# tzjtatata/Myriad

Measured on AMD Instinct MI355X. Metric: images/sec fine-tune step (Vicuna-7B + LoRA-style adapters, 224px), higher is better.
Workload: dtype bf16

## Files before the change

include/myriad_hip.h:

```cpp
#ifndef MYRIAD_HIP_H
#define MYRIAD_HIP_H
#include <stdint.h>

#ifdef __cplusplus
extern "C" {
#endif

typedef struct ihipStream_t* mh_stream_t;

#define MH_OK 0
#define MH_ERR_ARG (-1)
#define MH_ERR_LAUNCH (-2)
#define MH_ERR_UNSUPPORTED (-3)

#define MH_GEMM_OUT_F32 1
#define MH_GEMM_GELU 2
#define MH_GEMM_REGSTAGE 4

int mh_gemm_bf16_nt(const void* A, int lda, const void* B, int ldb, void* C, int ldc, int M, int N, int K,
                    const float* bias, const float* residual, int ldr, int flags, float alpha, mh_stream_t s);

int mh_gemm_plan(int M, int N, int K, int flags, int* kernel, int* splits);

int mh_prof_start(int capacity, mh_stream_t s);
double mh_prof_overhead_ms(void);
int mh_prof_stop(int* meta, float* ms, int cap, mh_stream_t s);

int mh_gemm_residual_rmsnorm(const void* A, int lda, const void* B, int ldb, float* H, int ldh, const float* residual,
                             int ldr, const float* norm_w, float eps, void* Y, long ldy, int M, int N, int K,
                             mh_stream_t s);

int mh_gemm_residual_layernorm(const void* A, int lda, const void* B, int ldb, float* H, int ldh, const float* bias,
                               const float* residual, int ldr, const float* norm_w, const float* norm_b, float eps, void* Y,
                               int M, int N, int K, mh_stream_t s);
int mh_gemm_rmsnorm_bwd(const void* A, int lda, const void* B, int ldb, float* dy_buf, const float* x, const float* w,
                        const float* dres, float* dx, void* dx_bf16, int M, int N, int K, float eps, mh_stream_t s);
int mh_gemm_layernorm_bwd(const void* A, int lda, const void* B, int ldb, float* dy_buf, const float* x, const float* w,
                          const float* dres, float* dx, void* dx_bf16, float* dgamma, float* dbeta, int accumulate, float* ws,
                          long ws_floats, int M, int N, int K, float eps, mh_stream_t s);

int mh_set_workspace(void* ptr, long bytes);
int mh_set_stream_workspace(mh_stream_t stream, void* ptr, long bytes);
long mh_gemm_splitk_ws_floats(int M, int N, int splits);
int mh_gemm_bf16_nt_splitk(const void* A, int lda, const void* B, int ldb, float* C, int ldc, int M, int N, int K,
                           int splits, float* ws, mh_stream_t s);

int mh_attn_fwd(const void* q, const void* k, const void* v, void* o, float* lse, const float* bias,
                const int* kv_len, int B, int H, int Sq, int Sk, int D, long q_bs, int ldq, long k_bs, int ldk,
                long v_bs, int ldv, long o_bs, int ldo, float scale, int causal, mh_stream_t s);
int mh_attn_fwd_dropout(const void* q, const void* k, const void* v, void* o, float* lse, int B, int H, int Sq, int Sk, int D,
                        long q_bs, int ldq, long k_bs, int ldk, long v_bs, int ldv, long o_bs, int ldo, float scale,
                        float drop_p, unsigned long long seed, mh_stream_t s);
int mh_attn_bwd_dropout(const void* q, const void* k, const void* v, const void* o, const void* dout, const float* lse,
                        float* delta_ws, void* dq, void* dk, void* dv, int B, int H, int Sq, int Sk, int D, long q_bs, int ldq,
                        long k_bs, int ldk, long v_bs, int ldv, long o_bs, int ldo, long do_bs, int lddo, long dq_bs,
                        int lddq, long dk_bs, int lddk, long dv_bs, int lddv, float scale, float drop_p,
                        unsigned long long seed, mh_stream_t s);
int mh_attn_bwd(const void* q, const void* k, const void* v, const void* o, const void* dout, const float* lse,
                float* delta_ws , void* dq, void* dk, void* dv, const float* bias,
                const int* kv_len, int B, int H, int Sq, int Sk, int D, long q_bs, int ldq, long k_bs, int ldk,
                long v_bs, int ldv, long o_bs, int ldo, long do_bs, int lddo, long dq_bs, int lddq, long dk_bs,
                int lddk, long dv_bs, int lddv, float scale, int causal, mh_stream_t s);

int mh_attn_rope_supported(int S, int D);
int mh_attn_rope_fwd(const void* qkv, int ld, void* o, int ldo, float* lse, const int* pos, const float* cos_tab,
                     const float* sin_tab, const int* kv_len, int B, int H, int S, int D, float scale, mh_stream_t s);
int mh_attn_rope_bwd(const void* qkv, int ld, const void* o, int ldo, const void* dout, int ldd, const float* lse,
                     void* dqkv, const int* pos, const float* cos_tab, const float* sin_tab, const int* kv_len,
                     int B, int H, int S, int D, float scale, mh_stream_t s);
int mh_gemm_attn_rope_bwd(const void* A, int lda, const void* Bw, int ldb, void* do_buf, int K, const void* qkv,
                          int ld, const void* o, int ldo, const float* lse, void* dqkv, const int* pos,
                          const float* cos_tab, const float* sin_tab, const int* kv_len, int B, int H, int S,
                          int D, float scale, mh_stream_t s);

int mh_rmsnorm_fwd(const float* x, const float* w, void* y_bf16, long ldy, int M, int D, float eps, mh_stream_t s);
int mh_rmsnorm_bwd(const float* dy, const float* x, const float* w, const float* dres, float* dx, void* dx_bf16,
                   int M, int D, float eps, mh_stream_t s);
int mh_layernorm_fwd(const float* x, const float* w, const float* b, void* y_bf16, float* y_f32, int M, int D,
                     float eps, mh_stream_t s);
int mh_layernorm_bwd(const float* dy, const float* x, const float* w, const float* dres, float* dx, void* dx_bf16,
                     int M, int D, float eps, mh_stream_t s);
long mh_layernorm_param_grads_ws_floats(int M, int D);
int mh_layernorm_param_grads(const float* dy, const float* x, float* dgamma, float* dbeta, int M, int D, float eps,
                             int accumulate, float p_out, unsigned long long seed_out, float* ws, long ws_floats,
                             mh_stream_t s);
int mh_layernorm_fwd_dropout(const float* z, const float* res, const float* w, const float* b, float* x_out, void* y_bf16,
                             float* y_f32, int M, int D, float eps, float p_in, unsigned long long seed_in, float p_out,
                             unsigned long long seed_out, mh_stream_t s);
int mh_layernorm_bwd_dropout(const float* dy, const float* x, const float* w, float* dx, void* dz_bf16, int M, int D,
                             float eps, float p_in, unsigned long long seed_in, float p_out, unsigned long long seed_out,
                             mh_stream_t s);
int mh_dropout_keep_mask(float* out, long n, float p, unsigned long long seed, mh_stream_t s);
int mh_drop_path_residual_layernorm(const float* h, const float* y, const int* slot_in, int K_in, float scale, const float* w,
                                    const float* b, const int* slot_out, int K_out, float* h_out, void* xn_bf16, int B, int N,
                                    int D, float eps, mh_stream_t s);
int mh_drop_path_layernorm_bwd(const float* dy, const float* x, const float* w, const float* dres, const int* slot_in, int K_in,
                               const int* slot_out, int K_out, float out_scale, float* dx, void* dx_bf16, int B, int N, int D,
                               float eps, mh_stream_t s);
int mh_drop_path_gather_scale(const float* src, const int* slot_out, int K_out, float scale, void* dst_bf16, int B, int N, int D,
                              mh_stream_t s);
long mh_drop_path_param_grads_ws_floats(int K, int N, int D);
int mh_drop_path_layernorm_param_grads(const float* dy, const float* x, const int* slot_in, int K_in, float* dgamma, float* dbeta,
                                       int B, int N, int D, float eps, int accumulate, float* ws, long ws_floats, mh_stream_t s);
long mh_gemm_tn_wgrad_ws_floats(int M, int N, int K, int splits);
int mh_gemm_tn_wgrad_auto_splits(int M, int N, int K);
int mh_gemm_tn_wgrad(const void* dy, long lddy, const void* x, long ldx, float* out, long ldo, float* bias, int M, int N, int K,
                     int accumulate, int splits, float* ws, long ws_floats, mh_stream_t s);

int mh_rope_inplace(void* x, int ld, int col0, int n_tok, int n_heads, int head_dim, const int* pos,
                    const float* cos_tab, const float* sin_tab, float sign, mh_stream_t s);
int mh_silu_mul_fwd(const void* gu, void* h, int M, int I, mh_stream_t s);
int mh_silu_mul_bwd(const void* dh, const void* gu, void* dgu, int M, int I, mh_stream_t s);
int mh_silu_mul_fwd_blk(const void* gu, void* h, int M, int I, int blk, mh_stream_t s);
int mh_silu_mul_bwd_blk(const void* dh, const void* gu, void* dgu, int M, int I, int blk, mh_stream_t s);
int mh_gemm_swiglu_fwd(const void* X, int ldx, const void* Wgu, int ldw, void* gu, int ldgu, void* act, int ldact, int M,
                       int I, int K, mh_stream_t s);
int mh_gemm_swiglu_bwd(const void* dH, int lddh, const void* WdT, int ldw, const void* gu, int ldgu, void* dgu, int lddgu,
                       void* dact_buf, int M, int I, int K, mh_stream_t s);
int mh_gelu_fwd(const void* x, void* y, long n, mh_stream_t s);
int mh_gelu_bwd(const void* dy, const void* x, void* dx, long n, mh_stream_t s);
int mh_gemm_gelu_fwd(const void* X, int ldx, const void* W, int ldw, const float* bias, void* pre, int ldpre, void* act, int ldact,
                     int M, int N, int K, mh_stream_t s);
int mh_gemm_gelu_bwd(const void* dY, int lddy, const void* WT, int ldw, const void* pre, int ldpre, void* dpre, int lddpre,
                     void* dact_buf, int M, int N, int K, mh_stream_t s);

int mh_dropout_bf16(const void* x, long ldx, void* y, long ldy, long rows, int cols, float p, unsigned long long seed,
                    mh_stream_t s);
int mh_dropout_add_f32(const float* dy, long lddy, float* acc, long ldacc, long rows, int cols, float p,
                       unsigned long long seed, mh_stream_t s);

int mh_lora_down(const void* x, long ldx, const float* A, void* border, long ldo, int M, int D, int R2, float s, float p,
                 unsigned long long seed, mh_stream_t st);
int mh_lora_dx(const float* dx_ext, long ld, const float* A, float* out, int M, int D, int R2, float s, float p,
               unsigned long long seed, mh_stream_t st);
int mh_rmsnorm_lora_down(const float* h, long ldh, const float* norm_w, float eps, const float* A, void* x_ext, long ldx, int M,
                         int D, int R2, float s, mh_stream_t st);
int mh_gemm_lora_dx(const void* A, int lda, const void* Bw, int ldb, float* dx_ext_buf, const float* loraA, float* dxn,
                    float* border_out, int M, int D, int K, int R2, float s, float p, unsigned long long seed, mh_stream_t stream);
int mh_gemm_lora_rmsnorm_bwd(const void* A, int lda, const void* Bw, int ldb, float* dx_ext_buf, const float* loraA,
                             float* dxn_buf, float* border_out, const float* x, const float* w, const float* dres, float* dx,
                             void* dx_bf16, int M, int D, int K, int R2, float s, float p, unsigned long long seed, float eps,
                             mh_stream_t stream);
long mh_lora_wgrad_ws_floats(int D, int R2);
int mh_lora_wgrad(const void* x, long ldx, const float* dx_ext, long ldg, const void* dq, const void* dv, long ldq,
                  const void* border, long ldb, float* dA, float* dBq, float* dBv, float* ws, int M, int D, int R2,
                  float s, float p, unsigned long long seed, mh_stream_t st);
int mh_lora_refresh_border(const float* Bq, const float* Bv, void* ext, long ld_ext, void* extT, long ld_extT, int W,
                           int D, int r, mh_stream_t st);
int mh_lora_refresh_borders(const void* table, int n_layers, long ld_ext, long ld_extT, int W, int D, int r, mh_stream_t stream);

int mh_lowrank_fwd(const float* x, const float* A, const float* Bm, float* y, float* t, int M, int D, int R,
                   mh_stream_t s);
long mh_lowrank_bwd_ws_floats(int M, int D, int R);
int mh_lowrank_bwd(const float* dy, const float* x, const float* t, const float* A, const float* Bm, float* dA,
                   float* dB, float* dx, float* ws, int M, int D, int R, mh_stream_t s);

int mh_clamp_ce(const float* logits, long ldl, const long* labels, float* row_loss, void* dlogits_bf16, long ldd,
                int R, int V, float grad_scale, mh_stream_t s);
int mh_sum_f32(const float* x, float* out, long n, float scale, mh_stream_t s);
int mh_argmax_rows(const float* logits, long ldl, long* out, float* margin, int R, int V, int ban_id, mh_stream_t s);
int mh_argmax_pmax_rows(const float* logits, long ldl, long* out, float* margin, float* pmax, int R, int V, int ban_id,
                        float inv_temp, mh_stream_t s);
int mh_decode_record(const long* nxt, const float* margin, const float* pmax, float* rec, long* next_ids, int* step, int R,
                     mh_stream_t s);
int mh_decode_advance(const long* nxt, const float* margin, const float* pmax, float* rec, long* next_ids, int* step, int* pos,
                      int* kvlen, int R, mh_stream_t s);
int mh_sample_rows(const float* logits, long ldl, long* out, float* margin, float* pmax, int* kept, float* u_out, int R, int V,
                   int ban_id, const float* params, const unsigned long long* seed, const int* step, int t_add, mh_stream_t s);
int mh_repetition_penalty_rows(float* logits, long ldl, unsigned* seen, const long* prev_ids, int R, int V, const float* penalty,
                               mh_stream_t s);
int mh_decode_advance_kept(const long* nxt, const float* margin, const float* pmax, const int* kept, float* rec, long* next_ids,
                           int* step, int* pos, int* kvlen, int R, mh_stream_t s);
int mh_decode_advance_rows(const long* nxt, const float* margin, const float* pmax, float* rec, long* next_ids, int* step,
                           int* pos, int* kvlen, const int* live, int R, mh_stream_t s);
int mh_sample_rows_slots(const float* logits, long ldl, long* out, float* margin, float* pmax, int* kept, float* u_out, int R, int V,
                         const float* params, const unsigned long long* seed, const int* gen, const int* live, mh_stream_t s);
int mh_argmax_pmax_rows_slots(const float* logits, long ldl, long* out, float* margin, float* pmax, int R, int V, const float* params,
                              const int* gen, const int* live, mh_stream_t s);
int mh_repetition_penalty_rows_slots(float* logits, long ldl, unsigned* seen, const long* prev_ids, int R, int V, const float* penalty,
                                     const int* live, mh_stream_t s);
int mh_decode_advance_kept_rows(const long* nxt, const float* margin, const float* pmax, const int* kept, float* rec, long* next_ids,
                                int* step, int* pos, int* kvlen, int* gen, const int* live, int R, mh_stream_t s);
int mh_token_scores_rows(const float* logits, long ldl, const long* ids, const int* watch, float* out, long ldo, int R, int V,
                         const int* live, mh_stream_t s);

int mh_beam_topk(const float* logits, long ldl, const float* scores, float* part_s, int* part_i, float* out_s, int* out_i, int B,
                 int rpi, int nb, int V, int ban_id, int* pos, int* kvlen, int n_adv, mh_stream_t s);
int mh_beam_reorder_kv(void* const* caches, int L, int B, int nb, long T_cap, int C, const int* src, const int* lo, const int* hi,
                       mh_stream_t s);
int mh_beam_topk_items(const float* logits, long ldl, const float* scores, float* part_s, int* part_i, float* out_s, int* out_i, int G,
                       int nb, int V, const int* live, int* gen, const int* prm, int* pos, int* kvlen, mh_stream_t s);
int mh_beam_reorder_kv_items(void* const* caches, int L, int G, int nb, long T_cap, int C, const int* src, const int* lo,
                             const int* hi, const int* live, mh_stream_t s);
int mh_beam_sample_topk(const float* logits, long ldl, const float* scores, const unsigned* seen, float* part_k, float* part_a,
                        int* part_i, int* part_f, float* out_s, int* out_i, int* out_f, float* out_k, int B, int nb, int V,
                        int ban_id, int draw, const float* params, const unsigned long long* seed, int* step, int t_add, int* pos,
                        int* kvlen, int n_adv, mh_stream_t s);
int mh_beam_seen_update(unsigned* seen, const int* src, const long* ids, int B, int nb, int V, mh_stream_t s);
int mh_beam_sample_topk_items(const float* logits, long ldl, const float* scores, const unsigned* seen, float* part_k, float* part_a,
                              int* part_i, int* part_f, float* out_s, int* out_i, int* out_f, float* out_k, int G, int nb, int V,
                              int draw, const float* params, const unsigned long long* seed, const int* live, int* gen,
                              const int* bprm, int t_add, int* pos, int* kvlen, mh_stream_t s);
int mh_beam_seen_update_items(unsigned* seen, const int* src, const long* ids, int G, int nb, int V, const int* live, mh_stream_t s);

int mh_im2col_nhwc(const void* x, void* col, int B, int H, int W, int C, int kh, int kw, int pad, int Kpad,
                   mh_stream_t s);
int mh_col2im_nhwc(const void* dcol, float* dx, int B, int H, int W, int C, int kh, int kw, int pad, int Kpad,
                   mh_stream_t s);
int mh_relu_maxpool2_fwd(const void* y, int y_is_f32, long ldy, void* p, int B, int H, int W, int C, mh_stream_t s);
int mh_relu_maxpool2_bwd(const float* dp, const void* y, int y_is_f32, long ldy, void* dy, long lddy, int B, int H,
                         int W, int C, mh_stream_t s);
int mh_conv_pack_weight(const float* W, const float* bias, void* Wp, int Cout, int K, int Kpad, mh_stream_t s);
int mh_conv_unpack_grad(const float* dWp, float* dW, float* db, int Cout, int K, int Kpad, mh_stream_t s);

int mh_embed_gather(const void* table_bf16, const long* ids, const int* dst_rows, float* out, long n, int D, long ldo,
                    mh_stream_t s);
int mh_copy2d_f32(const float* src, long lds, float* dst, long ldd, long rows, int cols, int accumulate,
                  mh_stream_t s);
int mh_copy3d_f32(const float* src, long src_bstride, long lds, float* dst, long dst_bstride, long ldd, int nb,
                  long rows, int cols, int accumulate, mh_stream_t s);
int mh_gather_rows_f32_to_bf16(const float* src, long lds, const int* rows, void* dst, long n, int D, mh_stream_t s);
int mh_gather_rows_f32(const float* src, long lds, const int* rows, float* dst, long n, int D, mh_stream_t s);
int mh_gather_rows(const void* src, long lds, const int* rows, void* dst, long n, int D, int elem_bytes, mh_stream_t s);
int mh_expand_rows(const void* src, const int* inv, void* dst, long ldd, long M, int D, int elem_bytes, mh_stream_t s);
int mh_copy3d_bf16(const void* src, long src_bstride, long lds, void* dst, long dst_bstride, long ldd, int nb,
                   long rows, int cols, mh_stream_t s);
int mh_kv_append_bf16(const void* src, long ld_src, void* cache, long cache_bstride, long ld_cache, const int* pos_dev,
                      int B, int cols, mh_stream_t s);
int mh_rope_kv_append(void* qkv, long ld, int n_heads, int head_dim, const int* pos, const float* cos_tab,
                      const float* sin_tab, void* cache, long cache_bstride, long ld_cache, const int* pos_dev, int B,
                      mh_stream_t s);
int mh_add_i32(int* x, int n, int delta, mh_stream_t s);
long mh_gemv_pack_elems(int N, int K);
int mh_gemv_pack(const void* W, int ldb, int N, int K, void* out, mh_stream_t s);
// ... 183 lines not shown
```

myriad_amd/csrc/common.h:

```cpp
#pragma once
#include <hip/hip_runtime.h>
#include <stdint.h>

#define MH_OK 0
#define MH_ERR_ARG (-1)
#define MH_ERR_LAUNCH (-2)
#define MH_ERR_UNSUPPORTED (-3)

typedef unsigned short bf16_t;
typedef __attribute__((ext_vector_type(8))) short short8_t;
typedef __attribute__((ext_vector_type(4))) short short4_t;
typedef __attribute__((ext_vector_type(4))) float float4_t;
typedef __attribute__((ext_vector_type(16))) float float16_t;

#define MH_CHECK_LAUNCH()                                   \
  do {                                                      \
    hipError_t e__ = hipGetLastError();                     \
    if (e__ != hipSuccess) return MH_ERR_LAUNCH;            \
  } while (0)

#define MH_MAX_ALT_WS 4
struct MhScratch {
  float* ws;
  size_t bytes;
  float* alt[MH_MAX_ALT_WS];
  hipStream_t alt_stream[MH_MAX_ALT_WS];
};
extern MhScratch g_default_scratch;
extern MhScratch* g_scratch;

enum MhOpt {
  MH_OPT_SLAB_BF16 = 0,
  MH_OPT_GEMM_SKINNY,
  MH_OPT_SWIGLU_FUSED,
  MH_OPT_GELU_FUSED,
  MH_OPT_ATTN_BWD_SPLIT,
  MH_OPT_GEMM_ZERO_PAD,
  MH_OPT_GEMM256_IMPL,
  MH_OPT_LORA_NORM_FUSED,
  MH_OPT_ATTN_FULL,
  MH_OPT_LORA_WGRAD_MFMA,
  MH_OPT_GEMM_SKIP_PAD,
  MH_OPT_GEMM_SPLIT_XCD,
  MH_OPT_COUNT
};
int mh_opt(int id);

extern bool g_mh_prof_on;
void mh_prof_pre(hipStream_t s, int kernel, int M, int N, int K, int splits, int flags);
void mh_prof_post(hipStream_t s);

__device__ __forceinline__ float bf2f(bf16_t h) { return __uint_as_float(((unsigned)h) << 16); }

typedef __bf16 mh_bf2_t __attribute__((ext_vector_type(2)));
typedef float mh_f2_t __attribute__((ext_vector_type(2)));
__device__ __forceinline__ bf16_t f2bf_sw(float f) {
  unsigned u = __float_as_uint(f);
  if ((u & 0x7fffffffu) > 0x7f800000u) return (bf16_t)((u >> 16) | 0x40);
  u += 0x7fffu + ((u >> 16) & 1u);
  return (bf16_t)(u >> 16);
}
__device__ __forceinline__ bf16_t f2bf(float f) {
  const __bf16 b = (__bf16)f;
  return (bf16_t)__builtin_bit_cast(unsigned short, b);
}
__device__ __forceinline__ unsigned pack_bf2(float lo, float hi) {
  const mh_f2_t v = {lo, hi};
  const mh_bf2_t b = __builtin_convertvector(v, mh_bf2_t);
  return __builtin_bit_cast(unsigned, b);
}

__device__ __forceinline__ unsigned dropout_hash(unsigned long long seed, unsigned long long idx) {
  unsigned h = (unsigned)idx * 0x9E3779B1u + ((unsigned)seed ^ ((unsigned)(idx >> 32) * 0x85EBCA77u));
  h ^= (unsigned)(seed >> 32) & 0x7FFFFFFFu;
  h ^= h >> 16;
  h *= 0x85EBCA6Bu;
  h ^= h >> 13;
  h *= 0xC2B2AE35u;
  h ^= h >> 16;
  return h;
}
__device__ __forceinline__ unsigned dropout_hash2(unsigned h) {
  h = (h ^ 0x68E31DA4u) * 0x2C1B3C6Du;
  return h ^ (h >> 15);
}
__device__ __forceinline__ float dropout_keep(unsigned long long seed, unsigned long long idx, float p, float inv_keep) {
  if (p <= 0.f) return 1.f;
  unsigned h = dropout_hash(seed, idx);
  if (seed >> 63) h = dropout_hash2(h);
  const float u = (float)(h >> 8) * (1.0f / 16777216.0f);
  return u >= p ? inv_keep : 0.f;
}
__device__ __forceinline__ void dropout_keep_pair(unsigned long long seed, unsigned long long idx, float p, float inv_keep,
                                                  float& k0, float& k1) {
  if (p <= 0.f) { k0 = k1 = 1.f; return; }
  const unsigned h = dropout_hash(seed, idx);
  k0 = (float)(h >> 8) * (1.0f / 16777216.0f) >= p ? inv_keep : 0.f;
  k1 = (float)(dropout_hash2(h) >> 8) * (1.0f / 16777216.0f) >= p ? inv_keep : 0.f;
}

__device__ __forceinline__ float4_t slab_load4(const void* base, long idx, int slab_bf16) {
  if (slab_bf16) {
    const short4_t h = *reinterpret_cast<const short4_t*>(reinterpret_cast<const bf16_t*>(base) + idx);
    return (float4_t){bf2f((bf16_t)h[0]), bf2f((bf16_t)h[1]), bf2f((bf16_t)h[2]), bf2f((bf16_t)h[3])};
  }
  return *reinterpret_cast<const float4_t*>(reinterpret_cast<const float*>(base) + idx);
}

__device__ __forceinline__ float lora_dx_value(float base, float s, float acc, float kq, float accv, float kv) {
#pragma clang fp contract(off)
  return __builtin_fmaf(s, __builtin_fmaf(acc, kq, accv * kv), base);
}
__device__ __forceinline__ void rms_bwd_sums(float x, float w, float g, float& ss, float& dot) {
#pragma clang fp contract(off)
  ss = __builtin_fmaf(x, x, ss);
  dot = __builtin_fmaf(x * w, g, dot);
}
__device__ __forceinline__ float rms_bwd_value(float r, float w, float g, float x, float cc) {
#pragma clang fp contract(off)
  return __builtin_fmaf(-x, cc, (r * w) * g);
}

__device__ __forceinline__ float wave_sum(float v) {
#pragma unroll
  for (int o = 32; o > 0; o >>= 1) v += __shfl_xor(v, o, 64);
  return v;
}
__device__ __forceinline__ float wave_max(float v) {
#pragma unroll
  for (int o = 32; o > 0; o >>= 1) v = fmaxf(v, __shfl_xor(v, o, 64));
  return v;
}

template <int NW>
__device__ __forceinline__ float block_sum(float v, float* red) {
  v = wave_sum(v);
  if (NW == 1) return v;
  const int w = threadIdx.x >> 6, l = threadIdx.x & 63;
  __syncthreads();
  if (l == 0) red[w] = v;
  __syncthreads();
  float t = 0.f;
#pragma unroll
  for (int i = 0; i < NW; ++i) t += red[i];
  return t;
}
template <int NW>
__device__ __forceinline__ float block_max(float v, float* red) {
  v = wave_max(v);
  if (NW == 1) return v;
  const int w = threadIdx.x >> 6, l = threadIdx.x & 63;
  __syncthreads();
  if (l == 0) red[w] = v;
  __syncthreads();
  float t = red[0];
#pragma unroll
  for (int i = 1; i < NW; ++i) t = fmaxf(t, red[i]);
  return t;
}

__device__ __forceinline__ float mh_erfc_abs(float ax, float gauss ) {
  const float t = __builtin_amdgcn_rcpf(1.f + 0.3275911f * ax);
  const float poly = t * (0.254829592f + t * (-0.284496736f + t * (1.421413741f + t * (-1.453152027f + t * 1.061405429f))));
  return poly * gauss;
}
__device__ __forceinline__ float mh_norm_cdf(float u , float gauss) {
  const float half = 0.5f * mh_erfc_abs(fabsf(u), gauss);
  return u < 0.f ? half : 1.f - half;
}
__device__ __forceinline__ float gelu_erf(float x) {
  const float u = x * 0.70710678118654752440f;
  return x * mh_norm_cdf(u, __expf(-u * u));
}
__device__ __forceinline__ float gelu_erf_grad(float x) {
  const float u = x * 0.70710678118654752440f;
  const float g = __expf(-u * u);
  const float cdf = mh_norm_cdf(u, g);
  const float pdf = 0.39894228040143267794f * g;
  return cdf + x * pdf;
}
```

myriad_amd/csrc/norm.hip:

```cpp
#include "common.h"

#define NT 256
#define NW 4

__global__ __launch_bounds__(NT) void rmsnorm_fwd_kernel(const float* __restrict__ x, const float* __restrict__ w,
                                                         bf16_t* __restrict__ y, int D, long ldy, float eps) {
  __shared__ float red[NW];
  const size_t row = blockIdx.x;
  const float* xr = x + row * D;
  float ss = 0.f;
  for (int i = threadIdx.x * 4; i < D; i += NT * 4) {
    const float4_t v = *reinterpret_cast<const float4_t*>(xr + i);
    ss += v[0] * v[0] + v[1] * v[1] + v[2] * v[2] + v[3] * v[3];
  }
  ss = block_sum<NW>(ss, red);
  const float r = rsqrtf(ss / D + eps);
  for (int i = threadIdx.x * 4; i < D; i += NT * 4) {
    const float4_t v = *reinterpret_cast<const float4_t*>(xr + i);
    const float4_t g = *reinterpret_cast<const float4_t*>(w + i);
    uint2 pk;
    pk.x = pack_bf2(g[0] * (v[0] * r), g[1] * (v[1] * r));
    pk.y = pack_bf2(g[2] * (v[2] * r), g[3] * (v[3] * r));
    *reinterpret_cast<uint2*>(y + row * ldy + i) = pk;
  }
}

template <int NIT>
__global__ __launch_bounds__(NT, NIT <= 4 ? 5 : 2) void rmsnorm_bwd_kernel(const void* __restrict__ dy, int nslab, long slab, long ldy,
                                                         const float* __restrict__ x, const float* __restrict__ w,
                                                         const float* dres, float* dx, bf16_t* dx_bf, int D, float eps, int sbf) {
  __shared__ float red[2 * NW];
  const size_t row = blockIdx.x;
  const float* xr = x + row * D;
  const long g0 = (long)row * ldy;
  constexpr bool PRE = NIT <= 4;
  float4_t xv[NIT], gv[NIT], dv[PRE ? NIT : 1];
  float ss = 0.f, dot = 0.f;
#pragma unroll
  for (int c = 0; c < NIT; ++c) {
    const int i = threadIdx.x * 4 + c * NT * 4;
    if (i < D) {
      xv[c] = *reinterpret_cast<const float4_t*>(xr + i);
      if (PRE && dres) dv[c] = *reinterpret_cast<const float4_t*>(dres + row * D + i);
    }
  }
#pragma unroll
  for (int c = 0; c < NIT; ++c) {
    const int i = threadIdx.x * 4 + c * NT * 4;
    if (i < D) {
      float4_t g = slab_load4(dy, g0 + i, sbf);
      int k = 1;
      if (nslab > 4)
      for (; k + 4 <= nslab; k += 4) {
        float4_t p[4];
#pragma unroll
        for (int u = 0; u < 4; ++u) p[u] = slab_load4(dy, g0 + (long)(k + u) * slab + i, sbf);
#pragma unroll
        for (int u = 0; u < 4; ++u) { g[0] += p[u][0]; g[1] += p[u][1]; g[2] += p[u][2]; g[3] += p[u][3]; }
      }
      for (; k < nslab; ++k) {
        const float4_t p = slab_load4(dy, g0 + (long)k * slab + i, sbf);
        g[0] += p[0]; g[1] += p[1]; g[2] += p[2]; g[3] += p[3];
      }
      if (nslab > 1) { g[0] *= 1.0f; g[1] *= 1.0f; g[2] *= 1.0f; g[3] *= 1.0f; }
      gv[c] = g;
    }
  }
#pragma unroll
  for (int c = 0; c < NIT; ++c) {
    const int i = threadIdx.x * 4 + c * NT * 4;
    if (i < D) {
      const float4_t ww = *reinterpret_cast<const float4_t*>(w + i);
#pragma unroll
      for (int e = 0; e < 4; ++e) rms_bwd_sums(xv[c][e], ww[e], gv[c][e], ss, dot);
    }
  }
  ss = wave_sum(ss);
  dot = wave_sum(dot);
  {
    const int wv_ = threadIdx.x >> 6, l = threadIdx.x & 63;
    if (l == 0) { red[wv_] = ss; red[NW + wv_] = dot; }
    __syncthreads();
    float t = 0.f, u = 0.f;
#pragma unroll
    for (int i = 0; i < NW; ++i) { t += red[i]; u += red[NW + i]; }
    ss = t; dot = u;
  }
  const float r = rsqrtf(ss / D + eps);
  const float cc = r * r * r * dot / D;
#pragma unroll
  for (int c = 0; c < NIT; ++c) {
    const int i = threadIdx.x * 4 + c * NT * 4;
    if (i < D) {
      const float4_t ww = *reinterpret_cast<const float4_t*>(w + i);
      float4_t o;
#pragma unroll
      for (int e = 0; e < 4; ++e) o[e] = rms_bwd_value(r, ww[e], gv[c][e], xv[c][e], cc);
      if (dres) {
        const float4_t d = PRE ? dv[c] : *reinterpret_cast<const float4_t*>(dres + row * D + i);
#pragma unroll
        for (int e = 0; e < 4; ++e) o[e] += d[e];
      }
      if (dx) *reinterpret_cast<float4_t*>(dx + row * D + i) = o;
      if (dx_bf) {
        uint2 pk;
        pk.x = pack_bf2(o[0], o[1]);
        pk.y = pack_bf2(o[2], o[3]);
        *reinterpret_cast<uint2*>(dx_bf + row * D + i) = pk;
      }
    }
  }
}

__global__ __launch_bounds__(NT) void layernorm_fwd_kernel(const float* __restrict__ x, const float* __restrict__ w,
                                                           const float* __restrict__ b, bf16_t* y_bf, float* y_f32,
                                                           int D, float eps) {
  __shared__ float red[NW];
  const size_t row = blockIdx.x;
  const float* xr = x + row * D;
  float s = 0.f;
  for (int i = threadIdx.x * 4; i < D; i += NT * 4) {
    const float4_t v = *reinterpret_cast<const float4_t*>(xr + i);
    s += v[0] + v[1] + v[2] + v[3];
  }
  const float mean = block_sum<NW>(s, red) / D;
  float ss = 0.f;
  for (int i = threadIdx.x * 4; i < D; i += NT * 4) {
    const float4_t v = *reinterpret_cast<const float4_t*>(xr + i);
#pragma unroll
    for (int e = 0; e < 4; ++e) ss += (v[e] - mean) * (v[e] - mean);
  }
  const float r = rsqrtf(block_sum<NW>(ss, red) / D + eps);
  for (int i = threadIdx.x * 4; i < D; i += NT * 4) {
    const float4_t v = *reinterpret_cast<const float4_t*>(xr + i);
    const float4_t g = *reinterpret_cast<const float4_t*>(w + i);
    const float4_t bb = *reinterpret_cast<const float4_t*>(b + i);
    float4_t o;
#pragma unroll
    for (int e = 0; e < 4; ++e) o[e] = (v[e] - mean) * r * g[e] + bb[e];
    if (y_f32) *reinterpret_cast<float4_t*>(y_f32 + row * D + i) = o;
    if (y_bf) {
      uint2 pk;
      pk.x = pack_bf2(o[0], o[1]);
      pk.y = pack_bf2(o[2], o[3]);
      *reinterpret_cast<uint2*>(y_bf + row * D + i) = pk;
    }
  }
}

template <int NIT>
__global__ __launch_bounds__(NT) void layernorm_bwd_kernel(const void* __restrict__ dy, int nslab, long slab, long ldy,
                                                           const float* __restrict__ x, const float* __restrict__ w,
                                                           const float* dres, float* dx, bf16_t* dx_bf, float* dy_out,
                                                           int D, float eps, int sbf) {
  __shared__ float red[NW];
  const size_t row = blockIdx.x;
  const float* xr = x + row * D;
  const long g0 = (long)row * ldy;
  float4_t xv[NIT], gv[NIT];
  float s = 0.f;
#pragma unroll
  for (int c = 0; c < NIT; ++c) {
    const int i = threadIdx.x * 4 + c * NT * 4;
    if (i < D) {
      xv[c] = *reinterpret_cast<const float4_t*>(xr + i);
      float4_t g = slab_load4(dy, g0 + i, sbf);
      for (int k = 1; k < nslab; ++k) {
        const float4_t p = slab_load4(dy, g0 + (long)k * slab + i, sbf);
        g[0] += p[0]; g[1] += p[1]; g[2] += p[2]; g[3] += p[3];
      }
      gv[c] = g;
      if (dy_out) *reinterpret_cast<float4_t*>(dy_out + row * D + i) = g;
      const float4_t v = xv[c];
      s += v[0] + v[1] + v[2] + v[3];
    }
  }
  const float mean = block_sum<NW>(s, red) / D;
  float ss = 0.f;
#pragma unroll
  for (int c = 0; c < NIT; ++c) {
    const int i = threadIdx.x * 4 + c * NT * 4;
    if (i < D) {
      const float4_t v = xv[c];
#pragma unroll
      for (int e = 0; e < 4; ++e) ss += (v[e] - mean) * (v[e] - mean);
    }
  }
  const float r = rsqrtf(block_sum<NW>(ss, red) / D + eps);
  float sg = 0.f, sgx = 0.f;
#pragma unroll
  for (int c = 0; c < NIT; ++c) {
    const int i = threadIdx.x * 4 + c * NT * 4;
    if (i < D) {
      const float4_t v = xv[c];
      const float4_t g = gv[c];
      const float4_t ww = *reinterpret_cast<const float4_t*>(w + i);
#pragma unroll
      for (int e = 0; e < 4; ++e) {
        const float gg = g[e] * ww[e];
        sg += gg;
        sgx += gg * (v[e] - mean) * r;
      }
    }
  }
  sg = block_sum<NW>(sg, red) / D;
  sgx = block_sum<NW>(sgx, red) / D;
#pragma unroll
  for (int c = 0; c < NIT; ++c) {
    const int i = threadIdx.x * 4 + c * NT * 4;
    if (i < D) {
      const float4_t v = xv[c];
      const float4_t g = gv[c];
      const float4_t ww = *reinterpret_cast<const float4_t*>(w + i);
      float4_t o;
#pragma unroll
      for (int e = 0; e < 4; ++e) o[e] = r * (g[e] * ww[e] - sg - (v[e] - mean) * r * sgx);
      if (dres) {
        const float4_t d = *reinterpret_cast<const float4_t*>(dres + row * D + i);
#pragma unroll
        for (int e = 0; e < 4; ++e) o[e] += d[e];
      }
      if (dx) *reinterpret_cast<float4_t*>(dx + row * D + i) = o;
      if (dx_bf) {
        uint2 pk;
        pk.x = pack_bf2(o[0], o[1]);
        pk.y = pack_bf2(o[2], o[3]);
        *reinterpret_cast<uint2*>(dx_bf + row * D + i) = pk;
      }
    }
  }
}

extern "C" int mh_rmsnorm_fwd(const float* x, const float* w, void* y_bf16, long ldy, int M, int D, float eps,
                              hipStream_t stream) {
  if (M <= 0) return MH_OK;
  if (D % 4 || ldy % 4 || ldy < D) return MH_ERR_ARG;
  hipLaunchKernelGGL(rmsnorm_fwd_kernel, dim3(M), dim3(NT), 0, stream, x, w, (bf16_t*)y_bf16, D, ldy, eps);
  MH_CHECK_LAUNCH();
  return MH_OK;
}

int mh_launch_rmsnorm_bwd(const void* dy, int slab_bf16, int nslab, long slab, long ldy, const float* x, const float* w,
                          const float* dres, float* dx, void* dx_bf16, int M, int D, float eps, hipStream_t stream) {
  if (M <= 0) return MH_OK;
  if ((D % 4) || D > 8192 || (ldy % 4) || nslab < 1) return MH_ERR_ARG;
  if (D <= 4 * NT * 4)
    hipLaunchKernelGGL(rmsnorm_bwd_kernel<4>, dim3(M), dim3(NT), 0, stream, dy, nslab, slab, ldy, x, w, dres, dx, (bf16_t*)dx_bf16, D,
                       eps, slab_bf16);
  else
    hipLaunchKernelGGL(rmsnorm_bwd_kernel<8>, dim3(M), dim3(NT), 0, stream, dy, nslab, slab, ldy, x, w, dres, dx, (bf16_t*)dx_bf16, D,
                       eps, slab_bf16);
  MH_CHECK_LAUNCH();
  return MH_OK;
}

extern "C" int mh_rmsnorm_bwd(const float* dy, const float* x, const float* w, const float* dres, float* dx,
                              void* dx_bf16, int M, int D, float eps, hipStream_t stream) {
  if (M <= 0) return MH_OK;
  return mh_launch_rmsnorm_bwd(dy, 0, 1, 0, D, x, w, dres, dx, dx_bf16, M, D, eps, stream);
}

extern "C" int mh_layernorm_fwd(const float* x, const float* w, const float* b, void* y_bf16, float* y_f32, int M,
                                int D, float eps, hipStream_t stream) {
  if (M <= 0) return MH_OK;
  if (D % 4) return MH_ERR_ARG;
  hipLaunchKernelGGL(layernorm_fwd_kernel, dim3(M), dim3(NT), 0, stream, x, w, b, (bf16_t*)y_bf16, y_f32, D, eps);
  MH_CHECK_LAUNCH();
  return MH_OK;
}

int mh_launch_layernorm_bwd(const void* dy, int slab_bf16, int nslab, long slab, long ldy, const float* x, const float* w,
                            const float* dres, float* dx, void* dx_bf16, float* dy_out, int M, int D, float eps,
                            hipStream_t stream) {
  if (M <= 0) return MH_OK;
  if ((D % 4) || D > 8192 || (ldy % 4) || ldy < D || nslab < 1) return MH_ERR_ARG;
#define LNB_LAUNCH(NIT_)                                                                                                   \
  hipLaunchKernelGGL(layernorm_bwd_kernel<NIT_>, dim3(M), dim3(NT), 0, stream, dy, nslab, slab, ldy, x, w, dres, dx,        \
                     (bf16_t*)dx_bf16, dy_out, D, eps, slab_bf16)
  if (D <= 2 * NT * 4) LNB_LAUNCH(2);
  else if (D <= 4 * NT * 4) LNB_LAUNCH(4);
  else LNB_LAUNCH(8);
#undef LNB_LAUNCH
  MH_CHECK_LAUNCH();
  return MH_OK;
}

extern "C" int mh_layernorm_bwd(const float* dy, const float* x, const float* w, const float* dres, float* dx,
                                void* dx_bf16, int M, int D, float eps, hipStream_t stream) {
  if (M <= 0) return MH_OK;
  return mh_launch_layernorm_bwd(dy, 0, 1, 0, D, x, w, dres, dx, dx_bf16, nullptr, M, D, eps, stream);
}
```

myriad_amd/csrc/version.hip:

```cpp
#include "common.h"
#include <stdlib.h>
#include <string.h>
extern "C" const char* mh_version(void) { return "myriad_hip 0.1 (gfx950)"; }
extern "C" int mh_target_arch(void) { return 950; }

struct MhOptEntry { const char* name; const char* env; int def; int value; };
static MhOptEntry g_opts[MH_OPT_COUNT] = {
    {"slab_bf16", "MYRIAD_SLAB_BF16", 1, -1},
    {"gemm_skinny", "MYRIAD_GEMM_SKINNY", 1, -1},
    {"swiglu_fused", "MYRIAD_SWIGLU_FUSED", 1, -1},
    {"gelu_fused", "MYRIAD_GELU_FUSED", 1, -1},
    {"attn_bwd_split", "MYRIAD_ATTN_BWD_SPLIT", 1, -1},
    {"gemm_zero_pad", "MYRIAD_GEMM_ZERO_PAD", 1, -1},
    {"gemm256_impl", "MYRIAD_GEMM256_IMPL", 1, -1},
    {"lora_norm_fused", "MYRIAD_LORA_NORM_FUSED", 1, -1},
    {"attn_full", "MYRIAD_ATTN_FULL", 1, -1},
    {"lora_wgrad_mfma", "MYRIAD_LORA_WGRAD_MFMA", 1, -1},
    {"gemm_skip_pad", "MYRIAD_GEMM_SKIP_PAD", 1, -1},
    {"gemm_split_xcd", "MYRIAD_GEMM_SPLIT_XCD", 1, -1},
};

int mh_opt(int id) {
  MhOptEntry& o = g_opts[id];
  if (o.value < 0) {
    const char* e = getenv(o.env);
    o.value = e ? (e[0] == '0' ? 0 : 1) : o.def;
  }
  return o.value;
}

static int find_opt(const char* name) {
  if (!name) return -1;
  for (int i = 0; i < MH_OPT_COUNT; ++i)
    if (!strcmp(name, g_opts[i].name)) return i;
  return -1;
}
extern "C" int mh_get_option(const char* name) {
  const int i = find_opt(name);
  return i < 0 ? MH_ERR_ARG : mh_opt(i);
}
extern "C" int mh_set_option(const char* name, int value) {
  const int i = find_opt(name);
  if (i < 0 || (value != 0 && value != 1)) return MH_ERR_ARG;
  const int prev = mh_opt(i);
  g_opts[i].value = value;
  return prev;
}
```

Before: 212.9.

## Process one LayerNorm row per wavefront for small hidden sizes

```diff
diff --git a/include/myriad_hip.h b/include/myriad_hip.h
--- a/include/myriad_hip.h
+++ b/include/myriad_hip.h
@@ -80,6 +80,8 @@
                      float eps, mh_stream_t s);
 int mh_layernorm_bwd(const float* dy, const float* x, const float* w, const float* dres, float* dx, void* dx_bf16,
                      int M, int D, float eps, mh_stream_t s);
+int mh_layernorm_bwd_slabs(const void* dy, int slab_bf16, int nslab, long slab, long ldy, const float* x, const float* w,
+                           const float* dres, float* dx, void* dx_bf16, float* dy_out, int M, int D, float eps, mh_stream_t s);
 long mh_layernorm_param_grads_ws_floats(int M, int D);
 int mh_layernorm_param_grads(const float* dy, const float* x, float* dgamma, float* dbeta, int M, int D, float eps,
                              int accumulate, float p_out, unsigned long long seed_out, float* ws, long ws_floats,
diff --git a/myriad_amd/csrc/common.h b/myriad_amd/csrc/common.h
--- a/myriad_amd/csrc/common.h
+++ b/myriad_amd/csrc/common.h
@@ -42,6 +42,7 @@
   MH_OPT_LORA_WGRAD_MFMA,
   MH_OPT_GEMM_SKIP_PAD,
   MH_OPT_GEMM_SPLIT_XCD,
+  MH_OPT_NORM_ROW_WAVES,
   MH_OPT_COUNT
 };
 int mh_opt(int id);
@@ -120,6 +121,31 @@
 #pragma clang fp contract(off)
   return __builtin_fmaf(-x, cc, (r * w) * g);
 }
+__device__ __forceinline__ float mh_unfused(float v) {
+  asm("" : "+v"(v));
+  return v;
+}
+__device__ __forceinline__ float ln_sum4(float s, float4_t v) {
+  return s + (v[0] + v[1] + v[2] + v[3]);
+}
+__device__ __forceinline__ float ln_sq_acc(float ss, float v, float mean) {
+#pragma clang fp contract(off)
+  return ss + mh_unfused((v - mean) * (v - mean));
+}
+__device__ __forceinline__ float ln_fwd_value(float v, float mean, float r, float g, float b) {
+#pragma clang fp contract(off)
+  return __builtin_fmaf((v - mean) * r, g, b);
+}
+__device__ __forceinline__ void ln_bwd_sums(float g, float w, float v, float mean, float r, float& sg, float& sgx) {
+#pragma clang fp contract(off)
+  const float gg = mh_unfused(g * w);
+  sg = sg + gg;
+  sgx = sgx + mh_unfused(gg * (v - mean) * r);
+}
+__device__ __forceinline__ float ln_bwd_value(float r, float g, float w, float sg, float v, float mean, float sgx) {
+#pragma clang fp contract(off)
+  return mh_unfused(r * __builtin_fmaf(-((v - mean) * r), sgx, __builtin_fmaf(g, w, -sg)));
+}
 
 __device__ __forceinline__ float wave_sum(float v) {
 #pragma unroll
diff --git a/myriad_amd/csrc/norm.hip b/myriad_amd/csrc/norm.hip
--- a/myriad_amd/csrc/norm.hip
+++ b/myriad_amd/csrc/norm.hip
@@ -121,14 +121,14 @@
   float s = 0.f;
   for (int i = threadIdx.x * 4; i < D; i += NT * 4) {
     const float4_t v = *reinterpret_cast<const float4_t*>(xr + i);
-    s += v[0] + v[1] + v[2] + v[3];
+    s = ln_sum4(s, v);
   }
   const float mean = block_sum<NW>(s, red) / D;
   float ss = 0.f;
   for (int i = threadIdx.x * 4; i < D; i += NT * 4) {
     const float4_t v = *reinterpret_cast<const float4_t*>(xr + i);
 #pragma unroll
-    for (int e = 0; e < 4; ++e) ss += (v[e] - mean) * (v[e] - mean);
+    for (int e = 0; e < 4; ++e) ss = ln_sq_acc(ss, v[e], mean);
   }
   const float r = rsqrtf(block_sum<NW>(ss, red) / D + eps);
   for (int i = threadIdx.x * 4; i < D; i += NT * 4) {
@@ -137,13 +137,71 @@
     const float4_t bb = *reinterpret_cast<const float4_t*>(b + i);
     float4_t o;
 #pragma unroll
-    for (int e = 0; e < 4; ++e) o[e] = (v[e] - mean) * r * g[e] + bb[e];
+    for (int e = 0; e < 4; ++e) o[e] = ln_fwd_value(v[e], mean, r, g[e], bb[e]);
     if (y_f32) *reinterpret_cast<float4_t*>(y_f32 + row * D + i) = o;
     if (y_bf) {
       uint2 pk;
       pk.x = pack_bf2(o[0], o[1]);
       pk.y = pack_bf2(o[2], o[3]);
       *reinterpret_cast<uint2*>(y_bf + row * D + i) = pk;
+    }
+  }
+}
+
+#define LN_RW_SLOTS(s) _Pragma("unroll") for (int s = 0; s < NS; ++s)
+
+template <int NS>
+__device__ __forceinline__ float ln_rw_sum(const float (&p)[NW]) {
+  float t = 0.f;
+#pragma unroll
+  for (int j = 0; j < NW; ++j) t += j < NS ? wave_sum(p[j]) : 0.f;
+  return t;
+}
+
+template <int NS>
+__global__ __launch_bounds__(NT) void layernorm_fwd_rw_kernel(const float* __restrict__ x, const float* __restrict__ w,
+                                                              const float* __restrict__ b, bf16_t* y_bf, float* y_f32,
+                                                              int M, int D, float eps) {
+  const int lane = threadIdx.x & 63;
+  const size_t row = (size_t)blockIdx.x * NW + (threadIdx.x >> 6);
+  if (row >= (size_t)M) return;
+  const float* xr = x + row * D;
+  constexpr int L = NS - 1;
+  const bool okl = 256 * L + lane * 4 < D;
+  int idx[NS];
+  LN_RW_SLOTS(s) idx[s] = 256 * s + (s < L || okl ? lane * 4 : 0);
+  float4_t xv[NS], wv[NS], bv[NS];
+  LN_RW_SLOTS(s) {
+    xv[s] = *reinterpret_cast<const float4_t*>(xr + idx[s]);
+    wv[s] = *reinterpret_cast<const float4_t*>(w + idx[s]);
+    bv[s] = *reinterpret_cast<const float4_t*>(b + idx[s]);
+  }
+  float p[NW] = {0.f, 0.f, 0.f, 0.f};
+  LN_RW_SLOTS(s) {
+    const float t = ln_sum4(p[s & 3], xv[s]);
+    p[s & 3] = s < L || okl ? t : p[s & 3];
+  }
+  const float mean = ln_rw_sum<NS>(p) / D;
+  float q[NW] = {0.f, 0.f, 0.f, 0.f};
+  LN_RW_SLOTS(s) {
+    float t = q[s & 3];
+#pragma unroll
+    for (int e = 0; e < 4; ++e) t = ln_sq_acc(t, xv[s][e], mean);
+    q[s & 3] = s < L || okl ? t : q[s & 3];
+  }
+  const float r = rsqrtf(ln_rw_sum<NS>(q) / D + eps);
+  LN_RW_SLOTS(s) {
+    float4_t o;
+#pragma unroll
+    for (int e = 0; e < 4; ++e) o[e] = ln_fwd_value(xv[s][e], mean, r, wv[s][e], bv[s][e]);
+    if (s < L || okl) {
+      if (y_f32) *reinterpret_cast<float4_t*>(y_f32 + row * D + idx[s]) = o;
+      if (y_bf) {
+        uint2 pk;
+        pk.x = pack_bf2(o[0], o[1]);
+        pk.y = pack_bf2(o[2], o[3]);
+        *reinterpret_cast<uint2*>(y_bf + row * D + idx[s]) = pk;
+      }
     }
   }
 }
@@ -172,7 +230,7 @@
       gv[c] = g;
       if (dy_out) *reinterpret_cast<float4_t*>(dy_out + row * D + i) = g;
       const float4_t v = xv[c];
-      s += v[0] + v[1] + v[2] + v[3];
+      s = ln_sum4(s, v);
     }
   }
   const float mean = block_sum<NW>(s, red) / D;
@@ -183,7 +241,7 @@
     if (i < D) {
       const float4_t v = xv[c];
 #pragma unroll
-      for (int e = 0; e < 4; ++e) ss += (v[e] - mean) * (v[e] - mean);
+      for (int e = 0; e < 4; ++e) ss = ln_sq_acc(ss, v[e], mean);
     }
   }
   const float r = rsqrtf(block_sum<NW>(ss, red) / D + eps);
@@ -196,11 +254,7 @@
       const float4_t g = gv[c];
       const float4_t ww = *reinterpret_cast<const float4_t*>(w + i);
 #pragma unroll
-      for (int e = 0; e < 4; ++e) {
-        const float gg = g[e] * ww[e];
-        sg += gg;
-        sgx += gg * (v[e] - mean) * r;
-      }
+      for (int e = 0; e < 4; ++e) ln_bwd_sums(g[e], ww[e], v[e], mean, r, sg, sgx);
     }
   }
   sg = block_sum<NW>(sg, red) / D;
@@ -214,7 +268,7 @@
       const float4_t ww = *reinterpret_cast<const float4_t*>(w + i);
       float4_t o;
 #pragma unroll
-      for (int e = 0; e < 4; ++e) o[e] = r * (g[e] * ww[e] - sg - (v[e] - mean) * r * sgx);
+      for (int e = 0; e < 4; ++e) o[e] = ln_bwd_value(r, g[e], ww[e], sg, v[e], mean, sgx);
       if (dres) {
         const float4_t d = *reinterpret_cast<const float4_t*>(dres + row * D + i);
 #pragma unroll
@@ -230,6 +284,132 @@
     }
   }
 }
+
+template <int NS, int SBF>
+__device__ __forceinline__ void ln_rw_load_dy(float4_t (&gv)[NS], const void* dy, int nslab, long slab, long g0, const int (&idx)[NS]) {
+  int k = 1;
+  if (nslab >= 3) {
+    float4_t p[2][NS];
+    LN_RW_SLOTS(s) {
+      gv[s] = slab_load4(dy, g0 + idx[s], SBF);
+      p[0][s] = slab_load4(dy, g0 + slab + idx[s], SBF);
+      p[1][s] = slab_load4(dy, g0 + 2 * slab + idx[s], SBF);
+    }
+    LN_RW_SLOTS(s) {
+#pragma unroll
+      for (int u = 0; u < 2; ++u) {
+        const float4_t a = p[u][s];
+        gv[s][0] += a[0]; gv[s][1] += a[1]; gv[s][2] += a[2]; gv[s][3] += a[3];
+      }
+    }
+    k = 3;
+  } else {
+    LN_RW_SLOTS(s) gv[s] = slab_load4(dy, g0 + idx[s], SBF);
+  }
+  if (NS <= 4)
+    for (; k + 2 <= nslab; k += 2) {
+      float4_t p[2][NS];
+      LN_RW_SLOTS(s) {
+        p[0][s] = slab_load4(dy, g0 + (long)k * slab + idx[s], SBF);
+        p[1][s] = slab_load4(dy, g0 + (long)(k + 1) * slab + idx[s], SBF);
+      }
+      LN_RW_SLOTS(s) {
+#pragma unroll
+        for (int u = 0; u < 2; ++u) {
+          const float4_t a = p[u][s];
+          gv[s][0] += a[0]; gv[s][1] += a[1]; gv[s][2] += a[2]; gv[s][3] += a[3];
+        }
+      }
+    }
+  for (; k < nslab; ++k) {
+    float4_t p[NS];
+    LN_RW_SLOTS(s) p[s] = slab_load4(dy, g0 + (long)k * slab + idx[s], SBF);
+    LN_RW_SLOTS(s) { gv[s][0] += p[s][0]; gv[s][1] += p[s][1]; gv[s][2] += p[s][2]; gv[s][3] += p[s][3]; }
+  }
+}
+
+template <int NS>
+__global__ __launch_bounds__(NT) void layernorm_bwd_rw_kernel(const void* __restrict__ dy, int nslab, long slab, long ldy,
+                                                              const float* __restrict__ x, const float* __restrict__ w,
+                                                              const float* dres, float* dx, bf16_t* dx_bf, float* dy_out,
+                                                              int M, int D, float eps, int sbf) {
+  const int lane = threadIdx.x & 63;
+  const size_t row = (size_t)blockIdx.x * NW + (threadIdx.x >> 6);
+  if (row >= (size_t)M) return;
+  const float* xr = x + row * D;
+  const long g0 = (long)row * ldy;
+  constexpr int L = NS - 1;
+  const bool okl = 256 * L + lane * 4 < D;
+  int idx[NS];
+  LN_RW_SLOTS(s) idx[s] = 256 * s + (s < L || okl ? lane * 4 : 0);
+  float4_t xv[NS], gv[NS], wv[NS], dv[NS];
+  const float* dr = dres ? dres + row * D : xr;
+  LN_RW_SLOTS(s) {
+    xv[s] = *reinterpret_cast<const float4_t*>(xr + idx[s]);
+    wv[s] = *reinterpret_cast<const float4_t*>(w + idx[s]);
+    dv[s] = *reinterpret_cast<const float4_t*>(dr + idx[s]);
+  }
+  if (sbf) ln_rw_load_dy<NS, 1>(gv, dy, nslab, slab, g0, idx);
+  else ln_rw_load_dy<NS, 0>(gv, dy, nslab, slab, g0, idx);
+  if (dy_out) {
+    LN_RW_SLOTS(s) if (s < L || okl) *reinterpret_cast<float4_t*>(dy_out + row * D + idx[s]) = gv[s];
+  }
+  float p[NW] = {0.f, 0.f, 0.f, 0.f};
+  LN_RW_SLOTS(s) {
+    const float t = ln_sum4(p[s & 3], xv[s]);
+    p[s & 3] = s < L || okl ? t : p[s & 3];
+  }
+  const float mean = ln_rw_sum<NS>(p) / D;
+  float q[NW] = {0.f, 0.f, 0.f, 0.f};
+  LN_RW_SLOTS(s) {
+    float t = q[s & 3];
+#pragma unroll
+    for (int e = 0; e < 4; ++e) t = ln_sq_acc(t, xv[s][e], mean);
+    q[s & 3] = s < L || okl ? t : q[s & 3];
+  }
+  const float r = rsqrtf(ln_rw_sum<NS>(q) / D + eps);
+  float pg[NW] = {0.f, 0.f, 0.f, 0.f}, pgx[NW] = {0.f, 0.f, 0.f, 0.f};
+  LN_RW_SLOTS(s) {
+    float t = pg[s & 3], u = pgx[s & 3];
+#pragma unroll
+    for (int e = 0; e < 4; ++e) ln_bwd_sums(gv[s][e], wv[s][e], xv[s][e], mean, r, t, u);
+    pg[s & 3] = s < L || okl ? t : pg[s & 3];
+    pgx[s & 3] = s < L || okl ? u : pgx[s & 3];
+  }
+  const float sg = ln_rw_sum<NS>(pg) / D;
+  const float sgx = ln_rw_sum<NS>(pgx) / D;
+  LN_RW_SLOTS(s) {
+    float4_t o;
+#pragma unroll
+    for (int e = 0; e < 4; ++e) o[e] = ln_bwd_value(r, gv[s][e], wv[s][e], sg, xv[s][e], mean, sgx);
+    if (dres) {
+#pragma unroll
+      for (int e = 0; e < 4; ++e) o[e] += dv[s][e];
+    }
+    if (s < L || okl) {
+      if (dx) *reinterpret_cast<float4_t*>(dx + row * D + idx[s]) = o;
+      if (dx_bf) {
+        uint2 pk;
+        pk.x = pack_bf2(o[0], o[1]);
+        pk.y = pack_bf2(o[2], o[3]);
+        *reinterpret_cast<uint2*>(dx_bf + row * D + idx[s]) = pk;
+      }
+    }
+  }
+}
+#undef LN_RW_SLOTS
+#define LN_RW_MAX_D 2048
+#define LN_RW_DISPATCH(LAUNCH, D_)       \
+  switch (((D_) + 255) / 256) {          \
+    case 1: LAUNCH(1); break;            \
+    case 2: LAUNCH(2); break;            \
+    case 3: LAUNCH(3); break;            \
+    case 4: LAUNCH(4); break;            \
+    case 5: LAUNCH(5); break;            \
+    case 6: LAUNCH(6); break;            \
+    case 7: LAUNCH(7); break;            \
+    default: LAUNCH(8); break;           \
+  }
 
 extern "C" int mh_rmsnorm_fwd(const float* x, const float* w, void* y_bf16, long ldy, int M, int D, float eps,
                               hipStream_t stream) {
@@ -264,7 +444,14 @@
                                 int D, float eps, hipStream_t stream) {
   if (M <= 0) return MH_OK;
   if (D % 4) return MH_ERR_ARG;
-  hipLaunchKernelGGL(layernorm_fwd_kernel, dim3(M), dim3(NT), 0, stream, x, w, b, (bf16_t*)y_bf16, y_f32, D, eps);
+  if (D > 0 && D <= LN_RW_MAX_D && mh_opt(MH_OPT_NORM_ROW_WAVES)) {
+#define LNF_RW_LAUNCH(NS_)                                                                                                 \
+  hipLaunchKernelGGL(layernorm_fwd_rw_kernel<NS_>, dim3((M + NW - 1) / NW), dim3(NT), 0, stream, x, w, b, (bf16_t*)y_bf16,  \
+                     y_f32, M, D, eps)
+    LN_RW_DISPATCH(LNF_RW_LAUNCH, D);
+#undef LNF_RW_LAUNCH
+  } else
+    hipLaunchKernelGGL(layernorm_fwd_kernel, dim3(M), dim3(NT), 0, stream, x, w, b, (bf16_t*)y_bf16, y_f32, D, eps);
   MH_CHECK_LAUNCH();
   return MH_OK;
 }
@@ -277,14 +464,27 @@
 #define LNB_LAUNCH(NIT_)                                                                                                   \
   hipLaunchKernelGGL(layernorm_bwd_kernel<NIT_>, dim3(M), dim3(NT), 0, stream, dy, nslab, slab, ldy, x, w, dres, dx,        \
                      (bf16_t*)dx_bf16, dy_out, D, eps, slab_bf16)
-  if (D <= 2 * NT * 4) LNB_LAUNCH(2);
+#define LNB_RW_LAUNCH(NS_)                                                                                                 \
+  hipLaunchKernelGGL(layernorm_bwd_rw_kernel<NS_>, dim3((M + NW - 1) / NW), dim3(NT), 0, stream, dy, nslab, slab, ldy, x, w, \
+                     dres, dx, (bf16_t*)dx_bf16, dy_out, M, D, eps, slab_bf16)
+  if (D > 0 && D <= LN_RW_MAX_D && mh_opt(MH_OPT_NORM_ROW_WAVES)) {
+    LN_RW_DISPATCH(LNB_RW_LAUNCH, D);
+  } else if (D <= 2 * NT * 4) LNB_LAUNCH(2);
   else if (D <= 4 * NT * 4) LNB_LAUNCH(4);
   else LNB_LAUNCH(8);
+#undef LNB_RW_LAUNCH
 #undef LNB_LAUNCH
   MH_CHECK_LAUNCH();
   return MH_OK;
 }
 
+extern "C" int mh_layernorm_bwd_slabs(const void* dy, int slab_bf16, int nslab, long slab, long ldy, const float* x, const float* w,
+                                      const float* dres, float* dx, void* dx_bf16, float* dy_out, int M, int D, float eps,
+                                      hipStream_t stream) {
+  if (!dy || !x || !w || (nslab > 1 && (slab < (long)M * ldy || slab % 4))) return MH_ERR_ARG;
+  return mh_launch_layernorm_bwd(dy, slab_bf16 ? 1 : 0, nslab, slab, ldy, x, w, dres, dx, dx_bf16, dy_out, M, D, eps, stream);
+}
+
 extern "C" int mh_layernorm_bwd(const float* dy, const float* x, const float* w, const float* dres, float* dx,
                                 void* dx_bf16, int M, int D, float eps, hipStream_t stream) {
   if (M <= 0) return MH_OK;
diff --git a/myriad_amd/csrc/version.hip b/myriad_amd/csrc/version.hip
--- a/myriad_amd/csrc/version.hip
+++ b/myriad_amd/csrc/version.hip
@@ -18,6 +18,7 @@
     {"lora_wgrad_mfma", "MYRIAD_LORA_WGRAD_MFMA", 1, -1},
     {"gemm_skip_pad", "MYRIAD_GEMM_SKIP_PAD", 1, -1},
     {"gemm_split_xcd", "MYRIAD_GEMM_SPLIT_XCD", 1, -1},
+    {"norm_row_waves", "MYRIAD_NORM_ROW_WAVES", 1, -1},
 };
 
 int mh_opt(int id) {
```

Result: no change. 213.0 (median of 4 runs) (+0.0%).
